# adobe/3D-FM-GAN

Hardware: AMD Instinct MI355X
Metric: (photo,render) pairs/sec (higher is better)
Workload: dtype f32; 1 GPU; pairs1024: cfg4 shard: E_Tsr+E_W+E_W_Plus(18 styles) on 256^2 -> co-mod -> Generator(1024) forward, fp32, B=8/GPU; pairs_per_gpu=8, global_pairs=8, image_size=1024, parallelism=replicas x1 (batch-sharded, no collective), launch=eager, ranks=1, full=False

## Files before the change

3d-fm-gan_amd/csrc/modconv_bf16.hip:

```cpp
#include <type_traits>
#include "common.h"

typedef unsigned u32x2 __attribute__((ext_vector_type(2)));

namespace {

typedef short bf16x8 __attribute__((ext_vector_type(8)));
typedef unsigned u32x4 __attribute__((ext_vector_type(4)));

__device__ __forceinline__ unsigned pack_bf16(float lo, float hi) {
  unsigned r;
  asm("v_cvt_pk_bf16_f32 %0, %1, %2" : "=v"(r) : "v"(lo), "v"(hi));
  return r;
}
__device__ __forceinline__ float bf16_to_f32(unsigned short v) { return __uint_as_float((unsigned)v << 16); }

__global__ __launch_bounds__(256) void modconv_weight_to_bf16(const float* __restrict__ wt,
                                                              unsigned short* __restrict__ wtb, int K, int M, int ktaps) {
  const int Mp = (M + 31) / 32 * 32, chunks = (K + 15) / 16;
  const long long total = (long long)chunks * ktaps * 2 * Mp * 4;
  for (long long idx = (long long)blockIdx.x * blockDim.x + threadIdx.x; idx < total;
       idx += (long long)gridDim.x * blockDim.x) {
    const int jp = (int)(idx & 3);
    long long r = idx >> 2;
    const int m = (int)(r % Mp); r /= Mp;
    const int hh = (int)(r & 1); r >>= 1;
    const int t = (int)(r % ktaps);
    const int c = (int)(r / ktaps);
    float v[2];
#pragma unroll
    for (int e = 0; e < 2; ++e) {
      const int k = c * 16 + hh * 8 + jp * 2 + e;
      v[e] = (m < M && k < K) ? wt[((long long)k * ktaps + t) * M + m] : 0.f;
    }
    reinterpret_cast<unsigned*>(wtb)[idx] = pack_bf16(v[0], v[1]);
  }
}

struct BFParams {
  const float* in; const unsigned short* wt; const float* style; const float* demod; float* out;
  int batch, cin, cout, h, w, oh, ow;
  long long out_plane_stride; int out_row_stride;
  int gh, gw;
  int tiles_x, tiles_y, o_tiles, mp;
  const float* noise; const float* noise_weight; const float* bias;
  int noise_batch, fuse_act; float alpha, act_scale;
};

// ... 258 lines not shown
              }
            }
          }
        }
      }
    }
  };
  if (bstore) {
    if (actf) rows(std::true_type{}, std::true_type{}); else rows(std::false_type{}, std::true_type{});
  } else {
    if (actf) rows(std::true_type{}, std::false_type{}); else rows(std::false_type{}, std::false_type{});
  }
}

__global__ __launch_bounds__(256) void modconv_weight_to_bf16x3(const float* __restrict__ wt, unsigned* __restrict__ wtb,
                                                                int K, int M, int ktaps) {
  const int Mp = (M + 31) / 32 * 32, chunks = (K + 15) / 16;
  const long long per_piece = (long long)ktaps * 2 * Mp * 4;
  const long long total = (long long)chunks * per_piece;
  for (long long idx = (long long)blockIdx.x * blockDim.x + threadIdx.x; idx < total;
       idx += (long long)gridDim.x * blockDim.x) {
    const int c = (int)(idx / per_piece);
    long long r = idx - (long long)c * per_piece;
    const int jp = (int)(r & 3); r >>= 2;
    const int m = (int)(r % Mp); r /= Mp;
    const int hh = (int)(r & 1);
    const int t = (int)(r >> 1);
    float v[2];
#pragma unroll
    for (int e = 0; e < 2; ++e) {
      const int k = c * 16 + hh * 8 + jp * 2 + e;
      v[e] = (m < M && k < K) ? wt[((long long)k * ktaps + t) * M + m] : 0.f;
    }
    const unsigned h01 = pack_bf16(v[0], v[1]);
    const float r0 = v[0] - __uint_as_float(h01 << 16), r1 = v[1] - __uint_as_float(h01 & 0xffff0000u);
    const unsigned m01 = pack_bf16(r0, r1);
    const float s0 = r0 - __uint_as_float(m01 << 16), s1 = r1 - __uint_as_float(m01 & 0xffff0000u);
    const unsigned l01 = pack_bf16(s0, s1);
    const long long base = (long long)c * 3 * per_piece + (idx - (long long)c * per_piece);
    wtb[base] = h01; wtb[base + per_piece] = m01; wtb[base + 2 * per_piece] = l01;
  }
}

template <int MODE, int RNP>
__global__ __launch_bounds__(256, 2) void modconv_mfma_bf16x3(const BFParams p) {
  static_assert(MODE == 0 || MODE == 1, "forward modes only");
  using Tile = BFTile<3, MODE, 1, RNP>;
  constexpr int BM = Tile::BM, TH = Tile::TH, TW = Tile::TW, PH = Tile::PH, PWP = Tile::PWP;
  constexpr int PLANE = PH * PWP;
  constexpr int NPH = MODE == 1 ? 4 : 1;
  constexpr int NU = (PLANE + 255) / 256;
  constexpr int WQ1 = 9 * 2 * BM;
  constexpr int WQ = 3 * WQ1;
  static_assert(WQ % 64 == 0, "weight image = whole DMA pieces");
  constexpr int WPIECES = WQ / 64, NWP = (WPIECES + 3) / 4;
  extern __shared__ u32x4 smem_q[];
  u32x4* Ws = smem_q;
  u32x4* Xs = smem_q + WQ;

  const int tid = threadIdx.x, lane = tid & 63, wave = __builtin_amdgcn_readfirstlane(tid >> 6);
  const int l31 = lane & 31, khalf = lane >> 5;
  unsigned lb = xcd_remap(blockIdx.x, gridDim.x);
  const int o_tile = lb % p.o_tiles; lb /= p.o_tiles;
  const int tx_i = lb % p.tiles_x; lb /= p.tiles_x;
  const int ty_i = lb % p.tiles_y;
  const int b = lb / p.tiles_y;
  const int o0 = o_tile * BM, x0 = tx_i * TW, y0 = ty_i * TH;
  const int hw = p.h * p.w;
  const float* style_b = p.style + (long long)b * p.cin;

  f32x16 acc[RNP][NPH];
// ... 205 lines not shown
#pragma unroll
              for (int py = 0; py < 2; ++py) {
                u32x2 t;
                t.x = __float_as_uint(acc[g][py * 2][r] * dm_m[r]);
                t.y = __float_as_uint(acc[g][py * 2 + 1][r] * dm_m[r]);
                __builtin_amdgcn_raw_buffer_store_b64(t, rsrc_o, vof, so_m + (unsigned)((r & 3) + 8 * (r >> 2)) * dps4 + (unsigned)py * drs4, 0);
              }
            } else {
              if (!(vg && o < p.cout)) continue;
              float* dst = dpos + (long long)o * p.out_plane_stride;
#pragma unroll
              for (int py = 0; py < 2; ++py) {
                if (2 * py_ + py >= p.oh) continue;
                const float v0 = acc[g][py * 2][r] * dm_m[r], v1 = acc[g][py * 2 + 1][r] * dm_m[r];
                if (pair) {
                  f32x2_u t;
                  t.x = v0; t.y = v1;
                  *reinterpret_cast<f32x2_u*>(dst + (long long)py * p.out_row_stride) = t;
                } else {
                  dst[(long long)py * p.out_row_stride] = v0;
                }
              }
            }
          }
        }
      }
    }
  };
  if (bstore) {
    if (actf) rows(std::true_type{}, std::true_type{}); else rows(std::false_type{}, std::true_type{});
  } else {
    if (actf) rows(std::true_type{}, std::false_type{}); else rows(std::false_type{}, std::false_type{});
  }
}

template <int PIECES, int MODE, int RM, int RNP>
int launch_tile(BFParams& p, hipStream_t s) {
  using Tile = BFTile<PIECES, MODE, RM, RNP>;
  void (*kernel)(const BFParams);
  if constexpr (PIECES == 3) kernel = modconv_mfma_bf16x3<MODE, RNP>;
  else kernel = modconv_mfma_bf16<MODE, RM, RNP>;
  p.tiles_x = (p.gw + Tile::TW - 1) / Tile::TW;
  p.tiles_y = (p.gh + Tile::TH - 1) / Tile::TH;
  p.o_tiles = (p.cout + Tile::BM - 1) / Tile::BM;
  const long long blocks = (long long)p.o_tiles * p.tiles_x * p.tiles_y * p.batch;
  if (blocks > 0x7fffffffLL) return FMGAN_EOVERFLOW;
  static bool attr = false;
  if (Tile::LDS > 48 * 1024 && !attr) {
    (void)hipFuncSetAttribute((const void*)kernel, hipFuncAttributeMaxDynamicSharedMemorySize, (int)Tile::LDS);
    attr = true;
  }
  hipLaunchKernelGGL(kernel, dim3((unsigned)blocks), dim3(256), Tile::LDS, s, p);
  return fmgan_check_launch();
}

int modconv2d_bf(int pieces, const float* in, const void* wt, const float* style, const float* demod, float* out, int batch,
                 int cin, int cout, int h, int w, int mode, const float* noise, const float* noise_weight,
                 const float* bias, int noise_batch, int fuse_act, float alpha, float act_scale,
                 long long out_plane_stride, int out_row_stride, hipStream_t s) {
  if (batch < 0 || cin <= 0 || cout <= 0 || h <= 0 || w <= 0) return FMGAN_EINVAL;
  if (mode < 0 || mode > (pieces == 3 ? 1 : 2)) return FMGAN_EUNSUPPORTED;
  if (mode != 0 && fuse_act) return FMGAN_EUNSUPPORTED;
  if (batch == 0) return FMGAN_OK;
  if (!(pieces == 3 ? fmgan_modconv2d_bf16x3_supported : fmgan_modconv2d_bf16_supported)(batch, cin, cout, h, w, mode))
    return FMGAN_EUNSUPPORTED;
  if (!in || !wt || !style || !out) return FMGAN_EINVAL;
// ... 55 lines not shown

extern "C" int fmgan_modconv2d_bf16(const float* in, const void* wt_bf16, const float* style, const float* demod,
                                    float* out, int batch, int cin, int cout, int h, int w, int mode, const float* noise,
                                    const float* noise_weight, const float* bias, int noise_batch, int fuse_act,
                                    float alpha, float act_scale, long long out_plane_stride, int out_row_stride,
                                    void* stream) {
  return modconv2d_bf(1, in, wt_bf16, style, demod, out, batch, cin, cout, h, w, mode, noise, noise_weight, bias,
                      noise_batch, fuse_act, alpha, act_scale, out_plane_stride, out_row_stride, (hipStream_t)stream);
}

extern "C" long long fmgan_modconv_weight_bf16x3_bytes(int cin, int cout, int ktaps) {
  const long long one = fmgan_modconv_weight_bf16_bytes(cin, cout, ktaps);
  return one < 0 ? one : 3 * one;
}

extern "C" int fmgan_modconv_weight_to_bf16x3(const float* wt, void* wt_split, int cin, int cout, int ktaps, void* stream) {
  return weight_to_bf(3, wt, wt_split, cin, cout, ktaps, (hipStream_t)stream);
}

extern "C" int fmgan_modconv2d_bf16x3_supported(int batch, int cin, int cout, int h, int w, int mode) {
  if (mode != 0 && mode != 1) return 0;
  if (!fmgan_modconv2d_bf16_supported(batch, cin, cout, h, w, mode)) return 0;
  return (long long)(cin >> 4) * 54 * ((cout + 31) / 32 * 32) * 16 < 0xFFFFFFF0LL ? 1 : 0;
}

extern "C" int fmgan_modconv2d_bf16x3(const float* in, const void* wt_split, const float* style, const float* demod,
                                      float* out, int batch, int cin, int cout, int h, int w, int mode, const float* noise,
                                      const float* noise_weight, const float* bias, int noise_batch, int fuse_act,
                                      float alpha, float act_scale, long long out_plane_stride, int out_row_stride,
                                      void* stream) {
  return modconv2d_bf(3, in, wt_split, style, demod, out, batch, cin, cout, h, w, mode, noise, noise_weight, bias,
                      noise_batch, fuse_act, alpha, act_scale, out_plane_stride, out_row_stride, (hipStream_t)stream);
}
```

3d-fm-gan_amd/op/_native.py:

```python
import ctypes
import os

import torch

_HERE = os.path.dirname(os.path.abspath(__file__))
LIB_PATH = os.environ.get('FMGAN_LIB') or os.path.join(os.path.dirname(_HERE), 'csrc', 'libfmgan_hip.so')

F32, F64, F16 = 0, 1, 2
FMGAN_OK, FMGAN_EUNSUPPORTED = 0, -2
LPIPS_SIZE = 256
_DTYPES = {torch.float32: F32, torch.float64: F64, torch.float16: F16}

_lib = None

amp_fwd = torch.amp.custom_fwd(device_type='cuda', cast_inputs=torch.float32)
amp_bwd = torch.amp.custom_bwd(device_type='cuda')


def _sig(fn, argtypes, restype=ctypes.c_int):
    fn.argtypes = argtypes
    fn.restype = restype
    return fn


# ... 43 lines not shown
    _sig(L.fmgan_face_crop_fwd_f32, [vp] * 3 + [i] * 4 + [vp])
    _sig(L.fmgan_face_crop_bwd_f32, [vp] * 3 + [i] * 4 + [vp])
    _sig(L.fmgan_detector_input_f32, [vp, vp, i, ll, vp])
    _sig(L.fmgan_heatmap_distance_blocks, [i, ll])
    _sig(L.fmgan_heatmap_distance_fwd_f32, [vp] * 3 + [i, ll, vp])
    _sig(L.fmgan_heatmap_distance_bwd_f32, [vp] * 5 + [i, ll, vp])
    _sig(L.fmgan_landmark_decode_f32, [vp] * 5 + [i] * 4 + [vp])
    _sig(L.fmgan_lpips_distance_blocks, [i] * 3)
    _sig(L.fmgan_lpips_distance_f32, [vp] * 4 + [i, i, i, f, vp])
    _sig(L.fmgan_lpips_distance_backward_f32, [vp] * 6 + [i, i, i, f, vp])
    _sig(L.fmgan_bn_prelu_f32, [vp] * 5 + [f, vp, vp] + [vp] * 4 + [f, vp, vp] + [i] * 5 + [vp])
    _sig(L.fmgan_se_pool_chunks, [i] * 4)
    _sig(L.fmgan_se_pool_f32, [vp, vp] + [i] * 4 + [vp])
    _sig(L.fmgan_se_gate_f32, [vp, i, ll] + [vp] * 4 + [f] + [vp] * 3 + [i] * 3 + [vp])
    _sig(L.fmgan_ir_tail_f32, [vp] * 5 + [f, vp, vp] + [i] * 3 + [vp] * 4 + [f, vp] + [vp] * 4 + [f, vp] + [i] * 4 + [vp])
    _sig(L.fmgan_modconv_demod_f32, [vp] * 3 + [i] * 4 + [f, f, vp])
    _sig(L.fmgan_modconv_wsq_f32, [vp] * 2 + [i] * 3 + [vp])
    _sig(L.fmgan_modconv_demod_wsq_f32, [vp] * 3 + [i] * 3 + [f, f, vp])
    _sig(L.fmgan_equal_linear_f32, [vp] * 4 + [i] * 3 + [vp])
    _sig(L.fmgan_wino_weight_f32, [vp, vp, i, i, vp])
    _sig(L.fmgan_wino_input_f32, [vp] * 3 + [i] * 4 + [vp])
    _sig(L.fmgan_wino_output_f32, [vp] * 6 + [i] * 6 + [f, f, vp])
    _sig(L.fmgan_modconv_weight_prep_f32, [vp, vp, i, i, i, f, i, vp])
    _sig(L.fmgan_modconv2d_workspace_bytes, [i] * 6, ll)
    _sig(L.fmgan_modconv2d_f32, [vp] * 5 + [i] * 6 + [vp] * 3 + [i, i, f, f, ll, i, vp, ll, vp])
    _sig(L.fmgan_modconv_weight_bf16_bytes, [i] * 3, ll)
    _sig(L.fmgan_modconv_weight_to_bf16, [vp, vp, i, i, i, vp])
    _sig(L.fmgan_modconv2d_bf16_supported, [i] * 6)
    _sig(L.fmgan_modconv2d_bf16, [vp] * 5 + [i] * 6 + [vp] * 3 + [i, i, f, f, ll, i, vp])
    _sig(L.fmgan_modconv_weight_bf16x3_bytes, [i] * 3, ll)
    _sig(L.fmgan_modconv_weight_to_bf16x3, [vp, vp, i, i, i, vp])
    _sig(L.fmgan_modconv2d_bf16x3_supported, [i] * 6)
    _sig(L.fmgan_modconv2d_bf16x3, [vp] * 5 + [i] * 6 + [vp] * 3 + [i, i, f, f, ll, i, vp])
    _sig(L.fmgan_modconv2d_rgb_fusable, [i] * 5)
    _sig(L.fmgan_modconv2d_select, [i] * 8 + [ctypes.POINTER(i)] * 5)
    _sig(L.fmgan_modconv2d_tiles, [ctypes.POINTER(i), i])
    _sig(L.fmgan_torgb_weight_mod_f32, [vp] * 3 + [i] * 3 + [f, vp])
    _sig(L.fmgan_modconv2d_rgb_f32, [vp] * 5 + [i] * 5 + [vp] * 3 + [i, i, f, f] + [vp] * 4 + [i, vp])
    _sig(L.fmgan_modconv_wgrad_workspace_bytes, [i] * 5, ll)
    _sig(L.fmgan_modconv_wgrad_f32, [vp] * 5 + [i] * 5 + [f, vp, ll, vp])
    _sig(L.fmgan_modconv_wgrad_mode_workspace_bytes, [i] * 6, ll)
    _sig(L.fmgan_modconv_wgrad_mode_f32, [vp] * 5 + [i] * 6 + [f, vp, ll, vp])
    _sig(L.fmgan_images_to_tensor, [vp, vp, i, i, i, f, f, vp])
    _sig(L.fmgan_resize_output_size, [i, i, i, ctypes.POINTER(ctypes.c_int), ctypes.POINTER(ctypes.c_int)])
    _sig(L.fmgan_resize_plan_ints, [i] * 4, ll)
    _sig(L.fmgan_resize_plan, [i] * 4 + [vp, ll])
    _sig(L.fmgan_resize_bilinear_u8, [vp] * 4 + [i] * 5 + [f, f, vp])
    _sig(L.fmgan_tensor_to_images, [vp, vp, i, i, i, f, f, vp])
    _sig(L.fmgan_tiles_to_canvas, [vp, vp, ctypes.POINTER(i)] + [i] * 6 + [f, f, vp])
    _sig(L.fmgan_bank_gather, [vp] * 4 + [i] * 6 + [vp, ll, vp, ll, ll, i, i, ctypes.POINTER(i), i, vp, f, f, i, vp])
    _sig(L.fmgan_torgb_f32, [vp] * 6 + [i] * 4 + [f, vp])
    _sig(L.fmgan_torgb_backward_splits, [i] * 3)
    _sig(L.fmgan_torgb_backward_f32, [vp] * 6 + [i] * 4 + [f, vp])
    _sig(L.fmgan_refresh_entry_bytes, [])
    _sig(L.fmgan_weight_refresh_blocks, [i, i, i, i, ll], ll)
    _sig(L.fmgan_weight_refresh_f32, [vp, i, ll, vp])
    _sig(L.fmgan_style_bank_entry_bytes, [])
    _sig(L.fmgan_style_bank_f32, [vp, i, vp, vp, i, i, i, vp, vp])
    _sig(L.fmgan_demod_bank_f32, [vp, i, vp, i, vp, vp])
    if L.fmgan_abi_version() != 1:
        raise RuntimeError('libfmgan_hip.so ABI version mismatch')
    _lib = L
    return L


def check(status, what):
# ... 829 lines not shown


def modconv2d_winograd(x, wt, style, demod, noise=None, noise_weight=None, bias=None, fuse_act=False, alpha=0.2,
                       act_scale=2 ** 0.5, u=None):
    require_gpu(x, 'input')
    x, style = x.contiguous(), style.contiguous()
    b, cin, h, w = x.shape
    if (h | w) & 1:
        raise RuntimeError('modconv2d_winograd: H and W must be even')
    if u is None:
        u = wino_weight(wt)
    cout = u.shape[1]
    n = b * (h // 2) * (w // 2)
    v = torch.empty((16, cin, n), dtype=torch.float32, device=x.device)
    m = torch.empty((16, cout, n), dtype=torch.float32, device=x.device)
    out = torch.empty((b, cout, h, w), dtype=torch.float32, device=x.device)
    nz, nb = _noise_args(noise)
    with launching(x, 'modconv2d_winograd', (b, cin, cout, h, w, 0)) as stream:
        check(lib().fmgan_wino_input_f32(fp(x), fp(style), fp(v), b, cin, h, w, stream), 'wino_input')
        torch.bmm(u, v, out=m)
        st = lib().fmgan_wino_output_f32(fp(m), fp(demod), fp(nz), fp(noise_weight), fp(bias), fp(out), b, cout, h, w,
                                         nb, int(bool(fuse_act)), float(alpha), float(act_scale), stream)
    check(st, 'wino_output')
    return out


def modconv_weight_to_bf16x3(wt):
    cin, taps, cout = wt.shape
    nbytes = lib().fmgan_modconv_weight_bf16x3_bytes(cin, cout, taps)
    wts = torch.empty(nbytes // 2, dtype=torch.int16, device=wt.device)
    with on_device(wt) as stream:
        check(lib().fmgan_modconv_weight_to_bf16x3(fp(wt), ptr(wts), cin, cout, taps, stream), 'modconv_weight_to_bf16x3')
    return wts


def current_modconv_precision():
    return _mc_precision


def modconv2d(x, wt, style, demod, mode, noise=None, noise_weight=None, bias=None, fuse_act=False, alpha=0.2,
              act_scale=2 ** 0.5, strided_out=None, precision=None):
    require_gpu(x, 'input')
    x = x.contiguous()
    style = style.contiguous()
    b, cin, h, w = x.shape
    cout = wt.shape[2]
    oh, ow = (2 * h + 1, 2 * w + 1) if mode == 1 else (((h - 3) // 2 + 1, (w - 3) // 2 + 1) if mode == 2 else (h, w))
    if strided_out is None:
        out = torch.empty((b, cout, oh, ow), dtype=torch.float32, device=x.device)
        out_ptr, ops, ors = out.data_ptr(), 0, 0
    else:
        out = None
        out_ptr, ops, ors = strided_out
    nz, nb = _noise_args(noise)
    prec, L = precision or _mc_precision, lib()
    if prec == 'bf16x3' and L.fmgan_modconv2d_bf16x3_supported(b, cin, cout, h, w, mode):
        name, wtb, extra = 'modconv2d_bf16x3', modconv_weight_to_bf16x3(wt), ()
    elif prec == 'bf16' and L.fmgan_modconv2d_bf16_supported(b, cin, cout, h, w, mode):
        name, wtb, extra = 'modconv2d_bf16', modconv_weight_to_bf16(wt), ()
    else:
        ws_bytes = L.fmgan_modconv2d_workspace_bytes(b, cin, cout, h, w, mode)
        ws = torch.empty(ws_bytes // 4, dtype=torch.float32, device=x.device) if ws_bytes else None
        name, wtb, extra = 'modconv2d', None, (fp(ws), ws_bytes)
    launch = getattr(L, 'fmgan_' + name + ('_f32' if wtb is None else ''))
    with launching(x, name, (b, cin, cout, h, w, mode)) as stream:
        st = launch(fp(x), fp(wt) if wtb is None else ptr(wtb), fp(style), fp(demod), out_ptr, b, cin, cout, h, w, mode,
# ... 238 lines not shown
```

3d-fm-gan_amd/op/live_weights.py:

```python
import numpy as np
import torch

from . import _native

_ENTRY = np.dtype([('src', '<u8'), ('dst', '<u8'), ('dst2', '<u8'), ('n', '<i8'), ('kind', '<i4'), ('cout', '<i4'),
                   ('cin', '<i4'), ('ktaps', '<i4'), ('scale', '<f4'), ('block_begin', '<u4')])


def _check_layout():
    if _native.lib().fmgan_refresh_entry_bytes() != _ENTRY.itemsize:
        raise RuntimeError('fmgan_refresh_entry layout mismatch between libfmgan_hip.so and op/live_weights.py')


class LiveWeights:

    def __init__(self, root):
        self.root = root
        self.active = False
        self._key = None
        self._table = None
        self._blocks = 0
        self._n = 0
        self._buffers = []

    def __deepcopy__(self, memo):
        import copy
        new = LiveWeights.__new__(LiveWeights)
        memo[id(self)] = new
        new.__init__(copy.deepcopy(self.root, memo))
        return new

    def _sources(self):
# ... 52 lines not shown
            return False
        key = tuple((p.data_ptr(), p.device.index) for p in params)
        if key != self._key:
            self._build(lin, conv, key)
        with _native.on_device(self._table) as stream:
            _native.check(_native.lib().fmgan_weight_refresh_f32(self._table.data_ptr(), self._n, self._blocks, stream),
                          'weight_refresh')
        return True

    def fresh(self):
        return _Fresh(self)


class _Fresh:
    def __init__(self, lw):
        self.lw = lw

    def __enter__(self):
        self.prev = self.lw.active
        if not self.prev:
            self.lw.active = self.lw.refresh()
        return self.lw

    def __exit__(self, *exc):
        self.lw.active = self.prev
        return False


def live(module):
    lv = getattr(module, '_live', None)
    if lv is not None and lv[0].active and not torch.is_grad_enabled():
        return lv[1], lv[2]
    return None
```

3d-fm-gan_amd/psp_encoder_model/encoders/psp_encoders.py:

```python
import math
import os

import torch
import torch.nn.functional as F
from torch import nn
from torch.nn import BatchNorm2d, Conv2d, Module, Sequential

from . import helpers
from .helpers import PReLU, bottleneck_IR, bottleneck_IR_SE, get_blocks
from stylegan2 import EqualLinear
from op import fused_leaky_relu
from op.live_weights import LiveWeights
from Util.streams import overlap_ok, run_deferred, side_streams

HEAD_STREAMS = int(os.environ.get('FMGAN_PSP_STREAMS', '2'))
GROUP_HEADS = os.environ.get('FMGAN_PSP_GROUPED', '0') == '1'

_TAPS = {18: (3, 5, 7), 50: (6, 20, 23)}


class GradualStyleBlock(Module):

    def __init__(self, in_c, out_c, spatial):
        super().__init__()
        self.out_c = out_c
        self.spatial = spatial
        layers, c = [], in_c
        for _ in range(int(math.log2(spatial))):
            layers += [Conv2d(c, out_c, kernel_size=3, stride=2, padding=1), nn.LeakyReLU()]
            c = out_c
        self.convs = nn.Sequential(*layers)
        self.linear = EqualLinear(out_c, out_c, lr_mul=1)

    def forward(self, x):
        if x.is_cuda and x.dtype == torch.float32:
            for conv, act in zip(self.convs[0::2], self.convs[1::2]):
                y = F.conv2d(x, conv.weight, None, conv.stride, conv.padding)
                if y.is_contiguous(memory_format=torch.channels_last) and not y.is_contiguous():
                    n, c, h, w = y.shape
                    y = fused_leaky_relu(y.permute(0, 2, 3, 1).reshape(-1, c), conv.bias, act.negative_slope, 1.0)
                    x = y.view(n, h, w, c).permute(0, 3, 1, 2)
                else:
                    x = fused_leaky_relu(y, conv.bias, act.negative_slope, 1.0)
            return self.linear(x.reshape(-1, self.out_c))
        return self.linear(self.convs(x).reshape(-1, self.out_c))


class GradualStyleEncoder(Module):
    def __init__(self, num_layers, mode='ir', opts=None):
        super().__init__()
        assert num_layers in [18, 50, 100, 152], 'num_layers should be 18, 50, 100, or 152'
        assert mode in ['ir', 'ir_se'], 'mode should be ir or ir_se'
        self.num_layers = num_layers
        unit = bottleneck_IR if mode == 'ir' else bottleneck_IR_SE
        self.input_layer = Sequential(Conv2d(opts.input_nc, 64, (3, 3), 1, 1, bias=False), BatchNorm2d(64), PReLU(64))
        self.body = Sequential(*[unit(b.in_channel, b.depth, b.stride) for stage in get_blocks(num_layers) for b in stage])
        self.style_count = opts.n_styles
        self.coarse_ind = 3
        self.middle_ind = 7
        self.styles = nn.ModuleList()
        for i in range(self.style_count):
            spatial = 16 if i < self.coarse_ind else (32 if i < self.middle_ind else 64)
            self.styles.append(GradualStyleBlock(512, 512, spatial))
        self.latlayer1 = nn.Conv2d(256, 512, kernel_size=1, stride=1, padding=0)
        self.latlayer2 = nn.Conv2d(128, 512, kernel_size=1, stride=1, padding=0)
        self.channels_last = True
        self._cl_key = None
        self._live_weights = None
        self._flat = None
# ... 87 lines not shown
        fused = helpers.fused_body(self.input_layer, self.body, x, (t1, t2, t3))
        if fused is not None:
            x, feats = fused
        else:
            x = self.input_layer(x)
            feats = {}
            for i, unit in enumerate(self.body):
                x = unit(x)
                if i in (t1, t2, t3):
                    feats[i] = x
        c1, c2, c3 = feats[t1], feats[t2], feats[t3]
        if GROUP_HEADS and x.is_cuda and x.dtype == torch.float32 and not torch.is_grad_enabled():
            flat = self._flatten_heads()
            if HEAD_STREAMS > 1 and overlap_ok(x):
                streams = side_streams(x.device, HEAD_STREAMS, 'psp-heads')

                def level(k, feat):
                    wait, outs = run_deferred(streams[k % HEAD_STREAMS], self._grouped_heads, flat[k], feat)
                    return [(wait, o) for o in outs]
            else:
                def level(k, feat):
                    return [((lambda: None), o) for o in self._grouped_heads(flat[k], feat)]
            latents = level(0, c3)
            if len(flat) > 1:
                p2 = self._upsample_add(c3, self.latlayer1(c2))
                latents += level(1, p2)
            if len(flat) > 2:
                p1 = self._upsample_add(p2, self.latlayer2(c1))
                latents += level(2, p1)
            return latents
        if HEAD_STREAMS > 1 and overlap_ok(x):
            streams = side_streams(x.device, HEAD_STREAMS, 'psp-heads')

            def head(j, feat):
                return run_deferred(streams[j % HEAD_STREAMS], self.styles[j], feat)
        else:
            def head(j, feat):
                return (lambda: None), self.styles[j](feat)
        latents = [head(j, c3) for j in range(min(self.coarse_ind, self.style_count))]
        p2 = self._upsample_add(c3, self.latlayer1(c2))
        latents += [head(j, p2) for j in range(self.coarse_ind, min(self.middle_ind, self.style_count))]
        p1 = self._upsample_add(p2, self.latlayer2(c1))
        latents += [head(j, p1) for j in range(self.middle_ind, self.style_count)]
        return latents
```

include/fmgan_hip.h:

```cpp
#ifndef FMGAN_HIP_H
#define FMGAN_HIP_H

#ifdef __cplusplus
extern "C" {
#endif

#define FMGAN_ABI_VERSION 1

#define FMGAN_OK            0
#define FMGAN_EINVAL       -1
#define FMGAN_EUNSUPPORTED -2
#define FMGAN_ELAUNCH      -3
#define FMGAN_EOVERFLOW    -4

#define FMGAN_F32 0
#define FMGAN_F64 1
#define FMGAN_F16 2

int         fmgan_abi_version(void);
const char *fmgan_status_string(int status);

int fmgan_upfirdn2d_select(int dtype, int major, int in_h, int in_w, int minor,
                           int kernel_h, int kernel_w, int up_x, int up_y,
                           int down_x, int down_y, int pad_x0, int pad_x1,
// ... 169 lines not shown
int fmgan_style_bank_entry_bytes(void);
int fmgan_style_bank_f32(const fmgan_style_bank_entry *table_dev, int n_entries, const float *w, const float *wplus,
                         int wplus_batch, int batch, int style_dim, float *styles_out, void *stream);
int fmgan_demod_bank_f32(const fmgan_style_bank_entry *table_dev, int n_entries, const float *styles, int batch,
                         float *demod_out, void *stream);

long long fmgan_modconv2d_workspace_bytes(int batch, int cin, int cout, int h, int w, int mode);
int fmgan_modconv2d_f32(const float *in, const float *wt, const float *style,
                        const float *demod, float *out,
                        int batch, int cin, int cout, int h, int w, int mode,
                        const float *noise, const float *noise_weight, const float *bias,
                        int noise_batch, int fuse_act, float alpha, float act_scale,
                        long long out_plane_stride, int out_row_stride,
                        void *workspace, long long workspace_bytes, void *stream);

long long fmgan_modconv_weight_bf16_bytes(int cin, int cout, int ktaps);
int fmgan_modconv_weight_to_bf16(const float *wt, void *wt_bf16, int cin, int cout, int ktaps, void *stream);
int fmgan_modconv2d_bf16_supported(int batch, int cin, int cout, int h, int w, int mode);
int fmgan_modconv2d_bf16(const float *in, const void *wt_bf16, const float *style, const float *demod, float *out,
                         int batch, int cin, int cout, int h, int w, int mode,
                         const float *noise, const float *noise_weight, const float *bias,
                         int noise_batch, int fuse_act, float alpha, float act_scale,
                         long long out_plane_stride, int out_row_stride, void *stream);

long long fmgan_modconv_weight_bf16x3_bytes(int cin, int cout, int ktaps);
int fmgan_modconv_weight_to_bf16x3(const float *wt, void *wt_split, int cin, int cout, int ktaps, void *stream);
int fmgan_modconv2d_bf16x3_supported(int batch, int cin, int cout, int h, int w, int mode);
int fmgan_modconv2d_bf16x3(const float *in, const void *wt_split, const float *style, const float *demod, float *out,
                           int batch, int cin, int cout, int h, int w, int mode,
                           const float *noise, const float *noise_weight, const float *bias,
                           int noise_batch, int fuse_act, float alpha, float act_scale,
                           long long out_plane_stride, int out_row_stride, void *stream);

int fmgan_torgb_weight_mod_f32(const float *rgb_weight, const float *rgb_style, float *wmod,
                               int batch, int cout, int rgb_channels, float rgb_scale, void *stream);
int fmgan_modconv2d_rgb_fusable(int batch, int cin, int cout, int h, int w);
int fmgan_modconv2d_rgb_f32(const float *in, const float *wt, const float *style,
                            const float *demod, float *out,
                            int batch, int cin, int cout, int h, int w,
                            const float *noise, const float *noise_weight, const float *bias,
                            int noise_batch, int fuse_act, float alpha, float act_scale,
                            const float *rgb_wmod, const float *rgb_bias,
                            const float *rgb_skip, float *rgb_out, int rgb_channels, void *stream);

int fmgan_modconv2d_select(int batch, int cin, int cout, int h, int w, int mode, int rgb, int has_workspace,
                           int *cfg, int *variant, int *bm, int *bn, int *ksplit);
int fmgan_modconv2d_tiles(int *out, int cap);

long long fmgan_modconv_wgrad_workspace_bytes(int batch, int cin, int cout, int h, int w);
long long fmgan_modconv_wgrad_mode_workspace_bytes(int batch, int cin, int cout, int h, int w, int mode);
int fmgan_modconv_wgrad_mode_f32(const float *go, const float *demod, const float *x, const float *style,
                                 float *gw, int batch, int cin, int cout, int h, int w, int mode, float scale,
                                 void *workspace, long long workspace_bytes, void *stream);
int fmgan_modconv_wgrad_f32(const float *go, const float *demod, const float *x, const float *style,
                            float *gw, int batch, int cin, int cout, int h, int w, float scale,
                            void *workspace, long long workspace_bytes, void *stream);

int fmgan_torgb_f32(const float *in, const float *weight, const float *style,
                    const float *bias, const float *skip, float *out,
                    int batch, int cin, int cout, int hw, float scale, void *stream);

int fmgan_torgb_backward_splits(int batch, int cin, int hw);
int fmgan_torgb_backward_f32(const float *x, const float *grad_out, const float *weight, const float *style,
                             float *grad_x, float *m_partial, int batch, int cin, int cout, int hw, float scale,
                             void *stream);

// ... 25 lines not shown
```

Baseline: 398.9 pairs/s.

## Add bf16x3 MFMA stride-2 3x3 conv kernel for pSp style-head first convs

Adds a dedicated stride-2 3x3 convolution kernel that splits fp32 inputs and weights into three bf16 pieces and runs six MFMA products per tap. It fuses bias and leaky-ReLU and can write channels-last output. The pSp encoder's GradualStyleBlock heads now route their first conv through this kernel, caching the split weight per module. The point is to replace the fp32 F.conv2d path with matrix-core work while keeping near-fp32 accuracy, plus a slow scalar fallback for non-finite values. The weight splitter also gains clamping and NaN/Inf handling.

Measured after the change: 419.9 pairs/s, median of 6. 5.3% higher.

```diff
diff --git a/3d-fm-gan_amd/csrc/modconv_bf16.hip b/3d-fm-gan_amd/csrc/modconv_bf16.hip
--- a/3d-fm-gan_amd/csrc/modconv_bf16.hip
+++ b/3d-fm-gan_amd/csrc/modconv_bf16.hip
@@ -14,6 +14,7 @@
   return r;
 }
 __device__ __forceinline__ float bf16_to_f32(unsigned short v) { return __uint_as_float((unsigned)v << 16); }
+constexpr float BF16_MAX = 3.3895313892515355e38f;
 
 __global__ __launch_bounds__(256) void modconv_weight_to_bf16(const float* __restrict__ wt,
                                                               unsigned short* __restrict__ wtb, int K, int M, int ktaps) {
@@ -338,11 +339,20 @@
       const int k = c * 16 + hh * 8 + jp * 2 + e;
       v[e] = (m < M && k < K) ? wt[((long long)k * ktaps + t) * M + m] : 0.f;
     }
-    const unsigned h01 = pack_bf16(v[0], v[1]);
-    const float r0 = v[0] - __uint_as_float(h01 << 16), r1 = v[1] - __uint_as_float(h01 & 0xffff0000u);
-    const unsigned m01 = pack_bf16(r0, r1);
-    const float s0 = r0 - __uint_as_float(m01 << 16), s1 = r1 - __uint_as_float(m01 & 0xffff0000u);
-    const unsigned l01 = pack_bf16(s0, s1);
+    unsigned piece[3][2];
+#pragma unroll
+    for (int e = 0; e < 2; ++e) {
+      const float x = v[e];
+      const bool fin = (__float_as_uint(x) & 0x7f800000u) != 0x7f800000u;
+      const float xc = fin ? __builtin_amdgcn_fmed3f(x, -BF16_MAX, BF16_MAX) : x;
+      const unsigned hb = pack_bf16(xc, 0.f) & 0xffffu;
+      const float r = fin ? x - bf16_to_f32((unsigned short)hb) : 0.f;
+      const unsigned mb = pack_bf16(r, 0.f) & 0xffffu;
+      const float s = r - bf16_to_f32((unsigned short)mb);
+      piece[0][e] = hb; piece[1][e] = mb; piece[2][e] = pack_bf16(s, 0.f) & 0xffffu;
+    }
+    const unsigned h01 = piece[0][0] | (piece[0][1] << 16), m01 = piece[1][0] | (piece[1][1] << 16);
+    const unsigned l01 = piece[2][0] | (piece[2][1] << 16);
     const long long base = (long long)c * 3 * per_piece + (idx - (long long)c * per_piece);
     wtb[base] = h01; wtb[base + per_piece] = m01; wtb[base + 2 * per_piece] = l01;
   }
@@ -614,6 +624,272 @@
   } else {
     if (actf) rows(std::true_type{}, std::false_type{}); else rows(std::false_type{}, std::false_type{});
   }
+}
+
+struct S2Params {
+  const float* in; const unsigned short* wt; const float* bias; float* out;
+  int batch, cin, cout, h, w, oh, ow;
+  int tiles_x, tiles_y, o_tiles, mp;
+  float alpha;
+  int out_nhwc;
+};
+
+struct S2Tile {
+  static constexpr int BM = 64, TH = 4, TW = 32;
+  static constexpr int PH = 2 * (TH - 1) + 3, PWP = 2 * (TW - 1) + 3, EVEN = (PWP + 1) / 2;
+  static constexpr int PLANE = PH * PWP;
+  static constexpr size_t LDS = (size_t)(3 * 2 * PLANE) * 16;
+};
+
+bool s2_plan(S2Params& p) {
+  if (p.batch <= 0 || p.cin <= 0 || p.cout <= 0 || p.h <= 0 || p.w <= 0) return false;
+  p.oh = (p.h - 1) / 2 + 1; p.ow = (p.w - 1) / 2 + 1;
+  p.mp = (p.cout + 31) / 32 * 32;
+  p.tiles_x = (p.ow + S2Tile::TW - 1) / S2Tile::TW;
+  p.tiles_y = (p.oh + S2Tile::TH - 1) / S2Tile::TH;
+  p.o_tiles = (p.cout + S2Tile::BM - 1) / S2Tile::BM;
+  if ((long long)p.cin * p.h * p.w * 4 >= 0xFFFFFFF0LL) return false;
+  if ((long long)((p.cin + 15) / 16) * 54 * p.mp * 16 >= 0xFFFFFFF0LL) return false;
+  if ((long long)p.o_tiles * p.tiles_x * p.tiles_y * p.batch > 0x7fffffffLL) return false;
+  if ((long long)p.batch * p.cout * p.oh * p.ow > (1LL << 40)) return false;
+  return true;
+}
+
+__global__ __launch_bounds__(256, 2) void conv3x3s2_mfma_bf16x3(const S2Params p) {
+  using Tile = S2Tile;
+  constexpr int BM = Tile::BM, TH = Tile::TH, TW = Tile::TW, PWP = Tile::PWP, EVEN = Tile::EVEN, PLANE = Tile::PLANE;
+  constexpr int RNP = 2;
+  constexpr int NU = (PLANE + 255) / 256;
+  extern __shared__ u32x4 smem_q[];
+  u32x4* Xs = smem_q;
+
+  const int tid = threadIdx.x, lane = tid & 63, wave = __builtin_amdgcn_readfirstlane(tid >> 6);
+  const int l31 = lane & 31, khalf = lane >> 5, wm = wave & 1, wn = wave >> 1;
+  unsigned lb = xcd_remap(blockIdx.x, gridDim.x);
+  const int o_tile = lb % p.o_tiles; lb /= p.o_tiles;
+  const int tx_i = lb % p.tiles_x; lb /= p.tiles_x;
+  const int ty_i = lb % p.tiles_y;
+  const int b = lb / p.tiles_y;
+  const int o0 = o_tile * BM, x0 = tx_i * TW, y0 = ty_i * TH;
+  const int hw = p.h * p.w;
+  const float* in_b = p.in + (long long)b * p.cin * hw;
+
+  f32x16 acc[RNP], acc_lo[RNP];
+#pragma unroll
+  for (int g = 0; g < RNP; ++g)
+#pragma unroll
+    for (int r = 0; r < 16; ++r) { acc[g][r] = 0.f; acc_lo[g][r] = 0.f; }
+
+  constexpr unsigned PARK = 0xFFFFFFF0u;
+  const unsigned x_bytes = (unsigned)((long long)p.cin * hw * 4);
+  const unsigned mp16 = (unsigned)p.mp * 16u;
+  const unsigned w_bytes = (unsigned)((p.cin + 15) >> 4) * 54u * mp16;
+  const auto rsrc_x = __builtin_amdgcn_make_buffer_rsrc(const_cast<float*>(in_b), 0, x_bytes, 0x00020000);
+  const auto rsrc_w = __builtin_amdgcn_make_buffer_rsrc(const_cast<unsigned short*>(p.wt), 0, w_bytes, 0x00020000);
+  unsigned xvo[NU];
+#pragma unroll
+  for (int u = 0; u < NU; ++u) {
+    const int q = tid + 256 * u;
+    const int r = q / PWP, t = q - r * PWP;
+    const int c = t < EVEN ? 2 * t : 2 * (t - EVEN) + 1;
+    const int y = 2 * y0 + r - 1, x = 2 * x0 + c - 1;
+    xvo[u] = (q < PLANE && y >= 0 && y < p.h && x >= 0 && x < p.w) ? (unsigned)(y * p.w + x) * 4u : PARK;
+  }
+  const int arow = o0 + wm * 32 + l31;
+  const unsigned avo = arow < p.mp ? (unsigned)(khalf * p.mp + arow) * 16u : PARK;
+
+  float xv[NU][16];
+  auto issue_x = [&](int i0, int kc) {
+    const unsigned soff = i0 + kc < p.cin ? (unsigned)((i0 + kc) * hw * 4) : 0u;
+#pragma unroll
+    for (int u = 0; u < NU; ++u)
+      xv[u][kc] = __builtin_bit_cast(float, __builtin_amdgcn_raw_buffer_load_b32(rsrc_x, xvo[u], soff, 0));
+  };
+  float xflag = 0.f;
+  auto commit_x = [&](int i0) {
+    if (i0 + 16 > p.cin) {
+#pragma unroll
+      for (int kc = 0; kc < 16; ++kc)
+        if (i0 + kc >= p.cin) {
+#pragma unroll
+          for (int u = 0; u < NU; ++u) xv[u][kc] = 0.f;
+        }
+    }
+#pragma unroll
+    for (int u = 0; u < NU; ++u) {
+      const int q = tid + 256 * u;
+      if (q < PLANE) {
+#pragma unroll
+        for (int hh = 0; hh < 2; ++hh) {
+          u32x4 ph, pm, pl;
+          unsigned* qh = reinterpret_cast<unsigned*>(&ph);
+          unsigned* qm = reinterpret_cast<unsigned*>(&pm);
+          unsigned* ql = reinterpret_cast<unsigned*>(&pl);
+#pragma unroll
+          for (int e = 0; e < 4; ++e) {
+            const float v0 = xv[u][8 * hh + 2 * e], v1 = xv[u][8 * hh + 2 * e + 1];
+            xflag = __builtin_fmaf(v0, 0.f, xflag);
+            xflag = __builtin_fmaf(v1, 0.f, xflag);
+            const unsigned h01 = pack_bf16(__builtin_amdgcn_fmed3f(v0, -BF16_MAX, BF16_MAX),
+                                           __builtin_amdgcn_fmed3f(v1, -BF16_MAX, BF16_MAX));
+            const float r0 = v0 - __uint_as_float(h01 << 16), r1 = v1 - __uint_as_float(h01 & 0xffff0000u);
+            const unsigned m01 = pack_bf16(r0, r1);
+            const float s0 = r0 - __uint_as_float(m01 << 16), s1 = r1 - __uint_as_float(m01 & 0xffff0000u);
+            qh[e] = h01; qm[e] = m01; ql[e] = pack_bf16(s0, s1);
+          }
+          Xs[(0 * 2 + hh) * PLANE + q] = ph;
+          Xs[(1 * 2 + hh) * PLANE + q] = pm;
+          Xs[(2 * 2 + hh) * PLANE + q] = pl;
+        }
+      }
+    }
+  };
+
+  int pbase[RNP];
+#pragma unroll
+  for (int g = 0; g < RNP; ++g) pbase[g] = khalf * PLANE + 2 * (wn * RNP + g) * PWP + l31;
+
+  struct Ops { u32x4 a[3]; bf16x8 b[3][RNP]; };
+  auto fetch_a = [&](Ops& o, unsigned soff_chunk, int t) {
+#pragma unroll
+    for (int pc = 0; pc < 3; ++pc)
+      o.a[pc] = __builtin_bit_cast(u32x4, __builtin_amdgcn_raw_buffer_load_b128(rsrc_w, avo, soff_chunk + (unsigned)(pc * 18 + t * 2) * mp16, 0));
+  };
+  auto fetch_b = [&](Ops& o, int t) {
+    const int ky = t / 3, kx = t - 3 * ky;
+    const int off = ky * PWP + (kx & 1) * EVEN + (kx >> 1);
+#pragma unroll
+    for (int pc = 0; pc < 3; ++pc)
+#pragma unroll
+      for (int g = 0; g < RNP; ++g) o.b[pc][g] = __builtin_bit_cast(bf16x8, Xs[pc * 2 * PLANE + pbase[g] + off]);
+  };
+  unsigned wflag = 0;
+  constexpr int PA[6] = {0, 2, 1, 0, 1, 0}, PB[6] = {2, 0, 1, 1, 0, 0};
+
+  const int chunks = (p.cin + 15) >> 4;
+#pragma unroll
+  for (int kc = 0; kc < 16; ++kc) issue_x(0, kc);
+  for (int ch = 0; ch < chunks; ++ch) {
+    const unsigned soff_chunk = (unsigned)ch * 54u * mp16;
+    Ops ops[2];
+    fetch_a(ops[0], soff_chunk, 0);
+    __syncthreads();
+    commit_x(16 * ch);
+    __syncthreads();
+    __builtin_amdgcn_sched_barrier(0);
+    fetch_b(ops[0], 0);
+    const int i0n = ch + 1 < chunks ? 16 * (ch + 1) : 0;
+#pragma unroll
+    for (int t = 0; t < 9; ++t) {
+      __builtin_amdgcn_sched_barrier(0);
+      if (t + 1 < 9) {
+        fetch_a(ops[(t + 1) & 1], soff_chunk, t + 1);
+        __builtin_amdgcn_sched_barrier(0);
+        issue_x(i0n, 2 * t); issue_x(i0n, 2 * t + 1);
+        fetch_b(ops[(t + 1) & 1], t + 1);
+      }
+      __builtin_amdgcn_sched_barrier(0);
+      const Ops& o = ops[t & 1];
+#pragma unroll
+      for (int e = 0; e < 4; ++e) wflag |= ((o.a[0][e] & 0x7f807f80u) + 0x00800080u) & 0x80008000u;
+      __builtin_amdgcn_s_setprio(1);
+#pragma unroll
+      for (int q = 0; q < 6; ++q)
+#pragma unroll
+        for (int g = 0; g < RNP; ++g) {
+          f32x16& dst = q == 5 ? acc[g] : acc_lo[g];
+          dst = __builtin_amdgcn_mfma_f32_32x32x16_bf16(__builtin_bit_cast(bf16x8, o.a[PA[q]]), o.b[PB[q]][g], dst, 0, 0, 0);
+        }
+      __builtin_amdgcn_s_setprio(0);
+    }
+    __builtin_amdgcn_sched_barrier(0);
+  }
+#pragma unroll
+  for (int g = 0; g < RNP; ++g)
+#pragma unroll
+    for (int r = 0; r < 16; ++r) acc[g][r] = __fadd_rn(acc[g][r], acc_lo[g][r]);
+
+  float* out_b = p.out + (long long)b * p.cout * p.oh * p.ow;
+  const float alpha = p.alpha;
+  const long long ost_o = p.out_nhwc ? 1 : (long long)p.oh * p.ow, ost_p = p.out_nhwc ? p.cout : 1;
+  if (__syncthreads_or((xflag != xflag) | (wflag != 0u))) {
+    const int pp = tid & 127, oy = y0 + (pp >> 5), ox = x0 + (pp & 31);
+    if (oy >= p.oh || ox >= p.ow) return;
+    for (int oo = 0; oo < 32; ++oo) {
+      const int o = o0 + (tid >> 7) * 32 + oo;
+      if (o >= p.cout) return;
+      float s = 0.f;
+      for (int i = 0; i < p.cin; ++i) {
+        const long long slot0 = (long long)(i >> 4) * 54 * p.mp;
+        const int hh = (i >> 3) & 1, j = i & 7;
+        for (int t = 0; t < 9; ++t) {
+          const int y = 2 * oy + t / 3 - 1, x = 2 * ox + t % 3 - 1;
+          const float xin = (y >= 0 && y < p.h && x >= 0 && x < p.w) ? in_b[(long long)i * hw + y * p.w + x] : 0.f;
+          float wv = 0.f;
+#pragma unroll
+          for (int pc = 0; pc < 3; ++pc)
+            wv += bf16_to_f32(p.wt[((slot0 + (long long)(pc * 18 + t * 2 + hh) * p.mp + o) << 3) + j]);
+          s = __builtin_fmaf(wv, xin, s);
+        }
+      }
+      const float v = __fadd_rn(s, p.bias ? p.bias[o] : 0.f);
+      out_b[o * ost_o + ((long long)oy * p.ow + ox) * ost_p] = v > 0.f ? v : v * alpha;
+    }
+    return;
+  }
+
+  const int orow = o0 + wm * 32 + 4 * khalf;
+  float bias_r[16];
+#pragma unroll
+  for (int r = 0; r < 16; ++r) bias_r[r] = p.bias ? p.bias[min(orow + (r & 3) + 8 * (r >> 2), p.cout - 1)] : 0.f;
+#pragma unroll
+  for (int g = 0; g < RNP; ++g) {
+    const int py_ = y0 + wn * RNP + g, px_ = x0 + l31;
+    if (py_ >= p.oh || px_ >= p.ow) continue;
+    float* dpos = out_b + ((long long)py_ * p.ow + px_) * ost_p;
+    float v[16];
+#pragma unroll
+    for (int r = 0; r < 16; ++r) {
+      const float t = __fadd_rn(acc[g][r], bias_r[r]);
+      v[r] = t > 0.f ? t : t * alpha;
+    }
+    if (p.out_nhwc && (p.cout & 3) == 0) {
+#pragma unroll
+      for (int j = 0; j < 4; ++j) {
+        const int o = orow + 8 * j;
+        if (o < p.cout) {
+          f32x4 q4 = {v[4 * j], v[4 * j + 1], v[4 * j + 2], v[4 * j + 3]};
+          *reinterpret_cast<f32x4*>(dpos + o) = q4;
+        }
+      }
+    } else {
+#pragma unroll
+      for (int r = 0; r < 16; ++r) {
+        const int o = orow + (r & 3) + 8 * (r >> 2);
+        if (o < p.cout) dpos[o * ost_o] = v[r];
+      }
+    }
+  }
+}
+
+int conv3x3s2_bf16x3(const float* in, const void* wt, const float* bias, float* out, int batch, int cin, int cout, int h,
+                     int w, float alpha, int out_nhwc, hipStream_t s) {
+  if (batch < 0 || cin <= 0 || cout <= 0 || h <= 0 || w <= 0 || (out_nhwc != 0 && out_nhwc != 1)) return FMGAN_EINVAL;
+  if (batch == 0) return FMGAN_OK;
+  S2Params p{};
+  p.in = in; p.wt = (const unsigned short*)wt; p.bias = bias; p.out = out;
+  p.batch = batch; p.cin = cin; p.cout = cout; p.h = h; p.w = w; p.alpha = alpha; p.out_nhwc = out_nhwc;
+  if (!s2_plan(p)) return FMGAN_EUNSUPPORTED;
+  if (!in || !wt || !out) return FMGAN_EINVAL;
+  if (out_nhwc && (cout & 3) == 0 && ((uintptr_t)out & 15)) return FMGAN_EINVAL;
+  static bool attr = false;
+  if (!attr) {
+    (void)hipFuncSetAttribute((const void*)conv3x3s2_mfma_bf16x3, hipFuncAttributeMaxDynamicSharedMemorySize, (int)S2Tile::LDS);
+    attr = true;
+  }
+  const long long blocks = (long long)p.o_tiles * p.tiles_x * p.tiles_y * p.batch;
+  hipLaunchKernelGGL(conv3x3s2_mfma_bf16x3, dim3((unsigned)blocks), dim3(256), S2Tile::LDS, s, p);
+  return fmgan_check_launch();
 }
 
 template <int PIECES, int MODE, int RM, int RNP>
@@ -735,3 +1011,14 @@
   return modconv2d_bf(3, in, wt_split, style, demod, out, batch, cin, cout, h, w, mode, noise, noise_weight, bias,
                       noise_batch, fuse_act, alpha, act_scale, out_plane_stride, out_row_stride, (hipStream_t)stream);
 }
+
+extern "C" int fmgan_conv3x3s2_bf16x3_supported(int batch, int cin, int cout, int h, int w) {
+  S2Params p{};
+  p.batch = batch; p.cin = cin; p.cout = cout; p.h = h; p.w = w;
+  return s2_plan(p) ? 1 : 0;
+}
+
+extern "C" int fmgan_conv3x3s2_bf16x3_f32(const float* in, const void* wt_split, const float* bias, float* out, int batch,
+                                          int cin, int cout, int h, int w, float alpha, int out_nhwc, void* stream) {
+  return conv3x3s2_bf16x3(in, wt_split, bias, out, batch, cin, cout, h, w, alpha, out_nhwc, (hipStream_t)stream);
+}
diff --git a/3d-fm-gan_amd/op/_native.py b/3d-fm-gan_amd/op/_native.py
--- a/3d-fm-gan_amd/op/_native.py
+++ b/3d-fm-gan_amd/op/_native.py
@@ -99,6 +99,8 @@
     _sig(L.fmgan_modconv_weight_to_bf16x3, [vp, vp, i, i, i, vp])
     _sig(L.fmgan_modconv2d_bf16x3_supported, [i] * 6)
     _sig(L.fmgan_modconv2d_bf16x3, [vp] * 5 + [i] * 6 + [vp] * 3 + [i, i, f, f, ll, i, vp])
+    _sig(L.fmgan_conv3x3s2_bf16x3_supported, [i] * 5)
+    _sig(L.fmgan_conv3x3s2_bf16x3_f32, [vp] * 4 + [i] * 5 + [f, i, vp])
     _sig(L.fmgan_modconv2d_rgb_fusable, [i] * 5)
     _sig(L.fmgan_modconv2d_select, [i] * 8 + [ctypes.POINTER(i)] * 5)
     _sig(L.fmgan_modconv2d_tiles, [ctypes.POINTER(i), i])
@@ -994,6 +996,31 @@
     with on_device(wt) as stream:
         check(lib().fmgan_modconv_weight_to_bf16x3(fp(wt), ptr(wts), cin, cout, taps, stream), 'modconv_weight_to_bf16x3')
     return wts
+
+
+def conv_weight_to_bf16x3(weight):
+    require_gpu(weight, 'weight')
+    cout, cin, kh, kw = weight.shape
+    with launching(weight, 'conv_weight_bf16x3', (cout, cin, kh * kw)):
+        wt = weight.detach().permute(1, 2, 3, 0).reshape(cin, kh * kw, cout).contiguous()
+        return modconv_weight_to_bf16x3(wt)
+
+
+def conv3x3s2_bf16x3_supported(batch, cin, cout, h, w):
+    return bool(lib().fmgan_conv3x3s2_bf16x3_supported(int(batch), int(cin), int(cout), int(h), int(w)))
+
+
+def conv3x3s2_bf16x3(x, wts, bias, cout, alpha=0.01, channels_last=False):
+    require_gpu(x, 'input')
+    if not x.is_contiguous():
+        raise RuntimeError(f'conv3x3s2_bf16x3: input must be NCHW-contiguous, got strides {x.stride()}')
+    b, cin, h, w = x.shape
+    out = torch.empty((b, cout, (h - 1) // 2 + 1, (w - 1) // 2 + 1), dtype=torch.float32, device=x.device,
+                      memory_format=torch.channels_last if channels_last else torch.contiguous_format)
+    with launching(x, 'conv3x3s2_bf16x3', (b, cin, cout, h, w)) as stream:
+        st = lib().fmgan_conv3x3s2_bf16x3_f32(fp(x), ptr(wts), fp(bias), fp(out), b, cin, cout, h, w, float(alpha),
+                                              int(bool(channels_last)), stream)
+    return out if served(st, 'conv3x3s2_bf16x3') else None
 
 
 def current_modconv_precision():
diff --git a/3d-fm-gan_amd/op/live_weights.py b/3d-fm-gan_amd/op/live_weights.py
--- a/3d-fm-gan_amd/op/live_weights.py
+++ b/3d-fm-gan_amd/op/live_weights.py
@@ -1,3 +1,5 @@
+import weakref
+
 import numpy as np
 import torch
 
@@ -116,3 +118,29 @@
     if lv is not None and lv[0].active and not torch.is_grad_enabled():
         return lv[1], lv[2]
     return None
+
+
+_SPLIT = weakref.WeakKeyDictionary()
+
+
+def split_conv_weight(conv):
+    w = conv.weight
+    key = (w.data_ptr(), w._version, w.device, tuple(w.shape), tuple(w.stride()))
+    kept = _SPLIT.get(conv)
+    stream = torch.cuda.current_stream(w.device)
+    if kept is None or kept[0] != key:
+        img = _native.conv_weight_to_bf16x3(w)
+        built = torch.cuda.Event()
+        built.record(stream)
+        kept = (key, img, built, stream)
+        _SPLIT[conv] = kept
+    elif kept[3] != stream:
+        stream.wait_event(kept[2])
+    return kept[1]
+
+
+def drop_split_weight(conv=None):
+    if conv is None:
+        _SPLIT.clear()
+    else:
+        _SPLIT.pop(conv, None)
diff --git a/3d-fm-gan_amd/psp_encoder_model/encoders/psp_encoders.py b/3d-fm-gan_amd/psp_encoder_model/encoders/psp_encoders.py
--- a/3d-fm-gan_amd/psp_encoder_model/encoders/psp_encoders.py
+++ b/3d-fm-gan_amd/psp_encoder_model/encoders/psp_encoders.py
@@ -10,11 +10,16 @@
 from .helpers import PReLU, bottleneck_IR, bottleneck_IR_SE, get_blocks
 from stylegan2 import EqualLinear
 from op import fused_leaky_relu
-from op.live_weights import LiveWeights
+from op import _native
+from op.live_weights import LiveWeights, split_conv_weight
 from Util.streams import overlap_ok, run_deferred, side_streams
 
 HEAD_STREAMS = int(os.environ.get('FMGAN_PSP_STREAMS', '2'))
 GROUP_HEADS = os.environ.get('FMGAN_PSP_GROUPED', '0') == '1'
+
+HEADS_X3 = os.environ.get('FMGAN_PSP_HEADS_X3', '1') == '1'
+X3_MIN_OUT = 32
+X3_TAIL_CHANNELS_LAST = True
 
 _TAPS = {18: (3, 5, 7), 50: (6, 20, 23)}
 
@@ -32,9 +37,29 @@
         self.convs = nn.Sequential(*layers)
         self.linear = EqualLinear(out_c, out_c, lr_mul=1)
 
-    def forward(self, x):
+    def x3_serves(self, x):
+        if not (HEADS_X3 and x.is_cuda and x.dtype == torch.float32 and not torch.is_grad_enabled()):
+            return False
+        conv = self.convs[0]
+        if conv.weight.dtype != torch.float32 or conv.bias is None or (x.shape[3] - 1) // 2 + 1 < X3_MIN_OUT:
+            return False
+        return _native.conv3x3s2_bf16x3_supported(x.shape[0], conv.in_channels, conv.out_channels, x.shape[2], x.shape[3])
+
+    def _first_x3(self, x_nchw):
+        conv, act = self.convs[0], self.convs[1]
+        y = _native.conv3x3s2_bf16x3(x_nchw, split_conv_weight(conv), conv.bias, conv.out_channels, act.negative_slope,
+                                     channels_last=X3_TAIL_CHANNELS_LAST)
+        if y is None:
+            raise RuntimeError('conv3x3s2_bf16x3 declined a shape its query accepted')
+        return y
+
+    def forward(self, x, x_nchw=None):
         if x.is_cuda and x.dtype == torch.float32:
-            for conv, act in zip(self.convs[0::2], self.convs[1::2]):
+            convs = list(zip(self.convs[0::2], self.convs[1::2]))
+            if self.x3_serves(x):
+                x = self._first_x3(x.contiguous() if x_nchw is None else x_nchw)
+                convs = convs[1:]
+            for conv, act in convs:
                 y = F.conv2d(x, conv.weight, None, conv.stride, conv.padding)
                 if y.is_contiguous(memory_format=torch.channels_last) and not y.is_contiguous():
                     n, c, h, w = y.shape
@@ -188,14 +213,19 @@
         if HEAD_STREAMS > 1 and overlap_ok(x):
             streams = side_streams(x.device, HEAD_STREAMS, 'psp-heads')
 
-            def head(j, feat):
-                return run_deferred(streams[j % HEAD_STREAMS], self.styles[j], feat)
+            def head(j, feat, nchw):
+                return run_deferred(streams[j % HEAD_STREAMS], self.styles[j], feat, nchw)
         else:
-            def head(j, feat):
-                return (lambda: None), self.styles[j](feat)
-        latents = [head(j, c3) for j in range(min(self.coarse_ind, self.style_count))]
+            def head(j, feat, nchw):
+                return (lambda: None), self.styles[j](feat, nchw)
+
+        def level(js, feat):
+            js = list(js)
+            nchw = feat.contiguous() if any(self.styles[j].x3_serves(feat) for j in js) else None
+            return [head(j, feat, nchw) for j in js]
+        latents = level(range(min(self.coarse_ind, self.style_count)), c3)
         p2 = self._upsample_add(c3, self.latlayer1(c2))
-        latents += [head(j, p2) for j in range(self.coarse_ind, min(self.middle_ind, self.style_count))]
+        latents += level(range(self.coarse_ind, min(self.middle_ind, self.style_count)), p2)
         p1 = self._upsample_add(p2, self.latlayer2(c1))
-        latents += [head(j, p1) for j in range(self.middle_ind, self.style_count)]
+        latents += level(range(self.middle_ind, self.style_count), p1)
         return latents
diff --git a/include/fmgan_hip.h b/include/fmgan_hip.h
--- a/include/fmgan_hip.h
+++ b/include/fmgan_hip.h
@@ -225,6 +225,10 @@
                            int noise_batch, int fuse_act, float alpha, float act_scale,
                            long long out_plane_stride, int out_row_stride, void *stream);
 
+int fmgan_conv3x3s2_bf16x3_supported(int batch, int cin, int cout, int h, int w);
+int fmgan_conv3x3s2_bf16x3_f32(const float *in, const void *wt_split, const float *bias, float *out,
+                               int batch, int cin, int cout, int h, int w, float alpha, int out_nhwc, void *stream);
+
 int fmgan_torgb_weight_mod_f32(const float *rgb_weight, const float *rgb_style, float *wmod,
                                int batch, int cout, int rgb_channels, float rgb_scale, void *stream);
 int fmgan_modconv2d_rgb_fusable(int batch, int cin, int cout, int h, int w);
```
